# lbroseus/TALC

Measured on AMD Instinct MI355X. Metric: corrected long-read bases/sec (whole node); k-mer-probe HBM GB/s, higher is better.
Workload: dtype u8

## Files before the change

talc_amd/csrc/talc_capi.hip:

```cpp
#include <hip/hip_runtime.h>

#include <algorithm>
#include <atomic>
#include <chrono>
#include <cstdarg>
#include <cstdio>
#include <cstring>
#include <fstream>
#include <map>
#include <memory>
#include <mutex>
#include <sstream>
#include <string>
#include <vector>

#include "talc_common.h"
#include "talc_devmem.h"
#include "talc_hip.h"
#include "talc_kernels_build.h"
#include "talc_kernels_count.h"
#include "talc_kernels_edits.h"
#include "talc_kernels_pieces.h"
#include "talc_kernels_probe.h"
#include "talc_kernels_search.h"
// ... 910 lines not shown
}

int talc_ctx_get_map_timing(const talc_ctx* c, float* pack_map_ms, float* mask_case_ms) {
  if (!c) return fail(TALC_ERR_INVALID, "null context");
  if (pack_map_ms) *pack_map_ms = c->pack_map_ms;
  if (mask_case_ms) *mask_case_ms = c->mask_case_ms;
  return TALC_OK;
}

int talc_ctx_get_pieces_timing(const talc_ctx* c, float* count_ms, float* pack_ms) {
  if (!c) return fail(TALC_ERR_INVALID, "null context");
  if (count_ms) *count_ms = c->piece_count_ms;
  if (pack_ms) *pack_ms = c->piece_pack_ms;
  return TALC_OK;
}

int talc_ctx_get_solidity_timing(const talc_ctx* c, float* raw_ms, float* corrected_ms) {
  if (!c) return fail(TALC_ERR_INVALID, "null context");
  if (raw_ms) *raw_ms = c->sol_raw_ms;
  if (corrected_ms) *corrected_ms = c->sol_corr_ms;
  return TALC_OK;
}

int talc_ctx_get_timing(const talc_ctx* c, talc_timing* out) {
  if (!c || !out) return fail(TALC_ERR_INVALID, "null argument");
  *out = c->timing;
  return TALC_OK;
}

void talc_batch_destroy(talc_batch* b) { delete b; }

int talc_batch_create(talc_ctx* c, const char* bases, const uint64_t* offsets, uint32_t n_reads, talc_batch** out) {
  if (!c || !offsets || !out || (!bases && n_reads && offsets[n_reads] > 0)) return fail(TALC_ERR_INVALID, "null argument");
  HIPCHK(hipSetDevice(c->device));
  auto b = std::make_unique<talc_batch>();
  b->ctx = c; b->n_reads = n_reads;
  b->h_state.use_pool(&c->host_pool); b->h_dense_off.use_pool(&c->host_pool); b->h_seg_off.use_pool(&c->host_pool);
  b->h_offsets.assign(offsets, offsets + n_reads + 1);
  if (b->h_offsets[0] != 0) return fail(TALC_ERR_INVALID, "offsets[0] must be 0");
  b->n_bases = b->h_offsets[n_reads];
  const uint32_t K = c->p.k;
  b->h_koff.resize(n_reads + 1);
  b->h_regoff.resize(n_reads + 1);
  b->h_outoff.resize(n_reads + 1);
  uint64_t ko = 0, ro = 0, oo = 0;
  for (uint32_t r = 0; r < n_reads; ++r) {
    if (offsets[r + 1] < offsets[r]) return fail(TALC_ERR_INVALID, "offsets must be non-decreasing");
    const uint64_t L = offsets[r + 1] - offsets[r];
    if (L > 0x7fffff00ull) return fail(TALC_ERR_INVALID, "read %u too long", r);
    b->max_len = std::max<uint32_t>(b->max_len, (uint32_t)L);
    const uint64_t nk = L >= K ? L - K + 1 : 0;
    b->h_koff[r] = ko; ko += nk;
    b->h_regoff[r] = ro; ro += nk / 2 + 2;
    b->h_outoff[r] = oo; oo += out_capacity_for(L);
    for (uint64_t p = 0; p < nk; p += COV_TILE) { b->h_tile_read.push_back(r); b->h_tile_start.push_back((uint32_t)p); }
    for (uint64_t p = 0; p < L; p += 4096) { b->h_chunk_read.push_back(r); b->h_chunk_start.push_back((uint32_t)p); }
  }
  b->h_koff[n_reads] = ko; b->h_regoff[n_reads] = ro; b->h_outoff[n_reads] = oo;
  b->n_kmers = ko;
  hipStream_t s = c->stream;
  int rc;
  HIPCHK(b->d_raw.alloc(c->cache, std::max<uint64_t>(b->n_bases, 1)));
  HIPCHK(b->d_codes.alloc(c->cache, std::max<uint64_t>(b->n_bases, 1) + 64));
  if (b->n_bases) HIPCHK(hipMemcpyAsync(b->d_raw.get(), bases, b->n_bases, hipMemcpyHostToDevice, s));
  if ((rc = up(c, b->d_offsets, b->h_offsets, s))) return rc;
  if ((rc = up(c, b->d_koff, b->h_koff, s))) return rc;
  if ((rc = up(c, b->d_regoff, b->h_regoff, s))) return rc;
  if ((rc = up(c, b->d_outoff, b->h_outoff, s))) return rc;
  if ((rc = up(c, b->d_tile_read, b->h_tile_read, s))) return rc;
  if ((rc = up(c, b->d_tile_start, b->h_tile_start, s))) return rc;
  if ((rc = up(c, b->d_chunk_read, b->h_chunk_read, s))) return rc;
  if ((rc = up(c, b->d_chunk_start, b->h_chunk_start, s))) return rc;
  HIPCHK(b->d_order.alloc(c->cache, std::max<uint32_t>(n_reads, 1)));
  HIPCHK(b->d_cov.alloc(c->cache, std::max<uint64_t>(b->n_kmers, 1)));
  HIPCHK(b->d_covw.alloc(c->cache, cov_words_total(b->n_kmers, n_reads)));
  HIPCHK(b->d_nin.alloc(c->cache, std::max<uint32_t>(n_reads, 1)));
  HIPCHK(b->d_state.alloc(c->cache, std::max<uint32_t>(n_reads, 1)));
  HIPCHK(b->d_headcov.alloc(c->cache, std::max<uint32_t>(n_reads, 1) * (uint64_t)kHeadCov));
  HIPCHK(b->d_regions.alloc(c->cache, std::max<uint64_t>(ro, 1) * 3));
  HIPCHK(b->d_out.alloc(c->cache, std::max<uint64_t>(oo, 1)));
  HIPCHK(hipStreamSynchronize(s));
  *out = b.release();
  return TALC_OK;
}

uint64_t talc_batch_num_kmers(const talc_batch* b) { return b ? b->n_kmers : 0; }
uint64_t talc_batch_num_bases(const talc_batch* b) { return b ? b->n_bases : 0; }

static int launch_vote(talc_ctx* c, talc_batch* b) {
  HIPCHK(b->d_strand.ensure(c->cache, b->n_reads));
  HIPCHK(b->d_strand_flag.ensure(c->cache, b->n_reads));
  HIPCHK(hipEventRecord(c->ev[kEvVote0], c->stream));
  if (b->n_reads)
    hipLaunchKernelGGL(k_strand_vote, dim3(b->n_reads), dim3(64), 0, c->stream, c->view, b->d_raw.get(), b->d_offsets.get(), c->p.min_count, b->n_reads,
                       b->d_strand.get(), b->d_strand_flag.get());
  HIPCHK(hipGetLastError());
  HIPCHK(hipEventRecord(c->ev[kEvVote1], c->stream));
  c->votePending = true;
  b->holds.voted = true;
  return TALC_OK;
}
static int vote_time(talc_ctx* c) {
  if (!c->votePending) return TALC_OK;
  HIPCHK(hipEventElapsedTime(&c->vote_ms, c->ev[kEvVote0], c->ev[kEvVote1]));
  c->votePending = false;
  return TALC_OK;
}
// ... 700 lines not shown
```

talc_amd/csrc/talc_capi_correct.inc:

```

static uint32_t next_launch_stamp() {
  static std::atomic<uint32_t> launches{0};
  return 0x01000000u + (launches.fetch_add(1) & 0xFFFFFFu);
}
static void ensure_edge_boxes(talc_ctx* c, Stage& st) {
  const uint64_t gap = (uint64_t)c->p.max_border_length + 256;
  const uint32_t seqCap = (uint32_t)align_up((uint64_t)(2.2 * (double)gap) + 4ull * c->p.k + 64, 16);
  const uint64_t need = (uint64_t)st.n_slots * edge_box_bytes(seqCap) + (uint64_t)st.n_slots * 4;
  if (c->sw.edgeTasks == 0 || c->p.max_start_anchors < 2 || c->p.max_start_anchors > EDGE_BOX_ANCHORS ||
      seqCap > (1u << 16) || need > (1ull << 30)) {
    st.boxes.reset(); st.boxes_bytes = 0;
    return;
  }
  if (need > st.boxes_bytes || seqCap != st.box_seq_cap) {
    st.boxes.reset(); st.boxes_bytes = 0;
    if (st.boxes.alloc(need) != hipSuccess) { (void)hipGetLastError(); return; }
    st.boxes_bytes = need; st.box_seq_cap = seqCap;
  }
}

static int ensure_stage(talc_ctx* c, Stage& st, uint32_t maxLen, uint32_t scale, uint32_t n_work) {
  const SearchCaps caps = make_caps(maxLen, c->p.k, scale, scale == 1 ? c->sw.seqArena : 0, scale == 1 && c->sw.tinyCaps);
  hipDeviceProp_t prop;
  HIPCHK(hipGetDeviceProperties(&prop, c->device));
// ... 100 lines not shown
  hipStream_t s = c->stream;
  int rc;
  memset(&c->timing, 0, sizeof c->timing);
  c->timing.n_kmers = b->n_kmers; c->timing.n_bases = b->n_bases;
  if ((rc = prepare_strand(c, b))) return rc;
  HIPCHK(hipEventRecord(c->ev[kEvBegin], s));
  if (!b->holds.encoded && (rc = launch_encode(c, b))) return rc;
  HIPCHK(hipEventRecord(c->ev[kEvEncoded], s));
  if ((rc = launch_coverage(c, b))) return rc;
  HIPCHK(hipEventRecord(c->ev[kEvCovered], s));
  HIPCHK(hipMemsetAsync(batch_stats(c), 0, kBatchStatsWords * sizeof(uint32_t), s));
  if (b->n_reads)
    hipLaunchKernelGGL(k_structure, dim3(b->n_reads), dim3(64), 0, s, c->dp, c->view, b->d_codes.get(), b->d_offsets.get(), b->d_koff.get(),
                       b->d_cov.get(), b->d_covw.get(), b->d_nin.get(), b->d_state.get(), b->d_regions.get(), b->d_regoff.get(), b->d_headcov.get(), b->n_reads, tb, traceRead, batch_stats(c));
  HIPCHK(hipGetLastError());
  HIPCHK(hipEventRecord(c->ev[kEvStructured], s));
  return TALC_OK;
}

static int order_queue(talc_ctx* c, talc_batch* b) {
  if (!b->n_reads) return TALC_OK;
  hipStream_t s = c->stream;
  uint32_t* const hist = c->d_hist.get();
  HIPCHK(hipMemsetAsync(hist, 0, kOrderBuckets * sizeof(uint32_t), s));
  const unsigned nb = (b->n_reads + kOrderBlock - 1) / kOrderBlock;
  hipLaunchKernelGGL(k_order_scale, dim3(1), dim3(64), 0, s, batch_stats(c));
  hipLaunchKernelGGL(k_order_hist, dim3(nb), dim3(kOrderBlock), 0, s, b->d_state.get(), b->n_reads, hist, batch_stats(c));
  hipLaunchKernelGGL(k_order_scan, dim3(1), dim3(kOrderBuckets), 0, s, hist);
  hipLaunchKernelGGL(k_order_scatter, dim3(nb), dim3(kOrderBlock), 0, s, b->d_state.get(), b->n_reads, hist, b->d_order.get(), batch_stats(c));
  HIPCHK(hipGetLastError());
  return TALC_OK;
}

static int launch_search(talc_ctx* c, talc_batch* b, const Stage& st, const uint32_t* d_work, uint32_t n_work, const TraceBuf& tb,
                         uint32_t traceRead, bool edgeTasks) {
  hipStream_t s = c->stream;
  HIPCHK(hipMemsetAsync(c->d_queue.get(), 0, kQueueWords * sizeof(uint32_t), s));
  const memcheck::Setting poison = memcheck::setting();
  if (poison.on && st.scratch_bytes) HIPCHK(hipMemsetAsync(st.scratch.get(), poison.byte, st.scratch_bytes, s));
  EdgeTaskArgs ea = {};
  ea.test = c->sw.edgeLane ? 0u : kTestNoEdgeLane;
  if (edgeTasks && st.boxes) {
    ea.boxes = st.boxes.get();
    ea.avail = (uint32_t*)(st.boxes.get() + (uint64_t)st.n_slots * edge_box_bytes(st.box_seq_cap));
    ea.seqCap = st.box_seq_cap;
    ea.minWeak = c->sw.edgeTaskMin; ea.heavy = c->sw.edgeTaskHeavy; ea.heavyRounds = c->sw.edgeTaskRounds;
    ea.lingerMod = c->sw.edgeLingerMod; ea.test |= c->sw.edgeRedo ? kTestEdgeRedo : 0u;
    ea.autoSwitch = c->sw.edgeTasks > 0 ? nullptr : batch_stats(c) + kStatBranching;
    if (poison.on) HIPCHK(hipMemsetAsync(ea.boxes, poison.byte, (uint64_t)st.n_slots * edge_box_bytes(st.box_seq_cap), s));
    HIPCHK(hipMemsetAsync(ea.avail, 0, (uint64_t)st.n_slots * 4, s));
  }
  hipLaunchKernelGGL(k_search, dim3(st.n_slots), dim3(64), 0, s, c->dp, c->view, st.caps, b->d_codes.get(), b->d_offsets.get(),
                     b->d_koff.get(), b->d_cov.get(), b->d_covw.get(), b->d_state.get(), b->d_regions.get(), b->d_regoff.get(), b->d_headcov.get(),
                     c->map ? b->d_regions.get() : nullptr, c->map ? b->d_mapedge.get() : nullptr, b->d_out.get(), b->d_outoff.get(), d_work,
                     n_work, c->d_queue.get(), st.scratch.get(), c->d_counters.get(), tb, traceRead, next_launch_stamp(), ea);
  HIPCHK(hipGetLastError());
  return TALC_OK;
}

static int search_first_pass(talc_ctx* c, talc_batch* b, const TraceBuf& tb, uint32_t traceRead) {
  hipStream_t s = c->stream;
  int rc;
  HIPCHK(hipMemsetAsync(c->d_counters.get(), 0, kCounterWords * sizeof(uint64_t), s));
  HIPCHK(hipMemsetAsync(c->d_counters.get() + kCntFirstStart, 0xFF, sizeof(uint64_t), s));
  HIPCHK(hipMemsetAsync(c->d_counters.get() + kCntQueueDry, 0xFF, sizeof(uint64_t), s));
  if (b->n_reads) {
    if ((rc = ensure_stage(c, c->stage, b->max_len, 1, b->n_reads))) return rc;
    ensure_edge_boxes(c, c->stage);
    if ((rc = launch_search(c, b, c->stage, b->d_order.get(), b->n_reads, tb, traceRead, true))) return rc;
  }
  HIPCHK(hipEventRecord(c->ev[kEvSearched], s));
  return TALC_OK;
}

static int emit_offsets(talc_ctx* c, talc_batch* b, bool map, const uint64_t** totals) {
  hipStream_t s = c->stream;
  const uint32_t n = b->n_reads, nb = emit_blocks(n);
  HIPCHK(b->d_emit.ensure(c->cache, nb + 1));
  HIPCHK(b->d_dense_off.ensure(c->cache, n + 1));
  if (map) HIPCHK(b->d_seg_off.ensure(c->cache, n + 1));
  EmitSum* const sums = b->d_emit.get();
  hipLaunchKernelGGL(k_emit_sums, dim3(nb), dim3(kEmitThreads), 0, s, b->d_state.get(), n, sums);
  hipLaunchKernelGGL(k_emit_offsets, dim3(nb), dim3(kEmitThreads), 0, s, b->d_state.get(), n, sums, b->d_dense_off.get(),
                     map ? b->d_seg_off.get() : nullptr, (unsigned long long*)(sums + nb));
  HIPCHK(hipGetLastError());
  HIPCHK(hipMemcpyAsync(c->h_land.data(), sums + nb, kTotWords * sizeof(uint64_t), hipMemcpyDeviceToHost, s));
  HIPCHK(hipStreamSynchronize(s));
  *totals = c->h_land.data();
  return TALC_OK;
}

static int search_retry_passes(talc_ctx* c, talc_batch* b, const TraceBuf& tb, uint32_t traceRead) {
  hipStream_t s = c->stream;
  int rc;
  std::vector<uint32_t> retry;
  for (uint32_t r = 0; r < b->n_reads; ++r) if (b->h_state[r].overflow) retry.push_back(r);
  c->timing.n_retried = (uint32_t)retry.size();
  HIPCHK(hipEventRecord(c->ev[kEvRetry0], s));
  for (uint32_t scale = 8; scale <= 64 && !retry.empty(); scale *= 8) {
    Stage big;
    if ((rc = ensure_stage(c, big, b->max_len, scale, (uint32_t)retry.size()))) {
      if (rc == TALC_ERR_NOMEM) break;
      return rc;
    }
    DevBuf<uint32_t> d_retry;
    if (d_retry.alloc(retry.size()) != hipSuccess) { (void)hipGetLastError(); break; }
    HIPCHK(hipMemcpyAsync(d_retry.get(), retry.data(), retry.size() * 4, hipMemcpyHostToDevice, s));
    for (uint32_t r : retry) {
      b->h_state[r].overflow = 0;
      HIPCHK(hipMemcpyAsync(b->d_state.get() + r, &b->h_state[r], sizeof(ReadState), hipMemcpyHostToDevice, s));
    }
    if ((rc = launch_search(c, b, big, d_retry.get(), (uint32_t)retry.size(), tb, traceRead, false))) return rc;
    if ((rc = fetch_states(c, b))) return rc;
    d_retry.reset(); big = Stage();
    std::vector<uint32_t> again;
    for (uint32_t r : retry) if (b->h_state[r].overflow) again.push_back(r);
    retry.swap(again);
  }
  HIPCHK(hipEventRecord(c->ev[kEvRetry1], s));
  return TALC_OK;
}

static int pack_dense(talc_ctx* c, talc_batch* b, uint64_t total) {
  hipStream_t s = c->stream;
  HIPCHK(b->d_dense.ensure(c->cache, total));
  if (b->n_reads)
    hipLaunchKernelGGL(k_pack, dim3(b->n_reads), dim3(256), 0, s, b->d_out.get(), b->d_outoff.get(), b->d_state.get(), b->d_dense_off.get(), b->d_dense.get(),
                       b->n_reads, c->p.reverse ? 1 : 0, b->rev_flags());
  HIPCHK(hipGetLastError());
  HIPCHK(hipEventRecord(c->ev[kEvEmitted], s));
  return TALC_OK;
}

static int pack_map(talc_ctx* c, talc_batch* b, uint64_t total) {
  hipStream_t s = c->stream;
  HIPCHK(b->d_segs.ensure(c->cache, total));
  if (b->n_reads)
    hipLaunchKernelGGL(k_pack_map, dim3(b->n_reads), dim3(64), 0, s, b->d_state.get(), b->d_regions.get(), b->d_regoff.get(), b->d_mapedge.get(),
                       b->d_offsets.get(), b->d_seg_off.get(), b->d_segs.get(), b->n_reads, c->p.k, c->p.reverse ? 1 : 0,
                       b->rev_flags());
  HIPCHK(hipGetLastError());
  HIPCHK(hipEventRecord(c->ev[kEvPackMap], s));
  return TALC_OK;
}

static int read_timing(talc_ctx* c, talc_batch* b, bool map, uint32_t n_failed, const uint64_t** counters) {
  hipStream_t s = c->stream;
  const uint32_t n = b->n_reads;
  int rc;
  if (!b->h_state.resize(n) || !b->h_dense_off.resize(n + 1) || (map && !b->h_seg_off.resize(n + 1)))
    return fail(TALC_ERR_NOMEM, "cannot allocate the host copies of %u reads' states and offsets", n);
  uint64_t* const land = c->h_land.data() + kTotWords;
  if (n) HIPCHK(hipMemcpyAsync(b->h_state.data(), b->d_state.get(), (size_t)n * sizeof(ReadState), hipMemcpyDeviceToHost, s));
  HIPCHK(hipMemcpyAsync(b->h_dense_off.data(), b->d_dense_off.get(), ((size_t)n + 1) * 8, hipMemcpyDeviceToHost, s));
  if (map) HIPCHK(hipMemcpyAsync(b->h_seg_off.data(), b->d_seg_off.get(), ((size_t)n + 1) * 8, hipMemcpyDeviceToHost, s));
  HIPCHK(hipMemcpyAsync(land, c->d_counters.get(), kCntWaveLog * sizeof(uint64_t), hipMemcpyDeviceToHost, s));
  HIPCHK(hipStreamSynchronize(s));
  if ((rc = read_stage_times(c, kEvEmitted))) return rc;
  c->timing.n_trail_steps = land[kCntSteps];
  c->timing.n_dp_cells = land[kCntCells];
  c->timing.n_failed = n_failed;
  if (c->sw.timing)
    fprintf(stderr, "[talc-lib] correction: host arrays page-locked: states %d, offsets %d, landing area %d\n", b->h_state.pinned() ? 1 : 0,
            b->h_dense_off.pinned() ? 1 : 0, c->h_land.pinned() ? 1 : 0);
  *counters = land;
  return TALC_OK;
}

static int run_pipeline(talc_ctx* c, talc_batch* b, TraceHost* th, uint32_t traceRead) {
  HIPCHK(hipSetDevice(c->device));
  int rc;
  b->holds.drop_results();
  const bool map = c->map;
  if (map) HIPCHK(b->d_mapedge.ensure(c->cache, 2ull * std::max<uint32_t>(b->n_reads, 1)));
  const TraceBuf tb = trace_buf(c, th);
  const uint64_t* counters = nullptr;
  const uint64_t* tot = nullptr;
  if ((rc = launch_structure(c, b, tb, traceRead))) return rc;
  if ((rc = order_queue(c, b))) return rc;
  if ((rc = search_first_pass(c, b, tb, traceRead))) return rc;
  HIPCHK(hipEventRecord(c->ev[kEvRetry0], c->stream));
  HIPCHK(hipEventRecord(c->ev[kEvRetry1], c->stream));
  if ((rc = emit_offsets(c, b, map, &tot))) return rc;
  if (tot[kTotOverflow]) {
    if ((rc = fetch_states(c, b))) return rc;
    if ((rc = search_retry_passes(c, b, tb, traceRead))) return rc;
    if ((rc = emit_offsets(c, b, map, &tot))) return rc;
  }
  const uint32_t n_failed = (uint32_t)tot[kTotOverflow];
  if ((rc = pack_dense(c, b, tot[kTotBytes]))) return rc;
  if (map && (rc = pack_map(c, b, tot[kTotSegs]))) return rc;
  if ((rc = read_timing(c, b, map, n_failed, &counters)) || (rc = vote_time(c))) return rc;
  if (map) HIPCHK(hipEventElapsedTime(&c->pack_map_ms, c->ev[kEvEmitted], c->ev[kEvPackMap]));
#ifdef TALC_PROF
  if ((rc = prof_report(c, b, counters))) return rc;
#endif
  b->holds.corrected = true; b->holds.mapped = map;
  if (c->timing.n_failed) {
    fail(TALC_WARN_READ_ERRORS, "%u read(s) exhausted the device scratch even in the retry pass (status TALC_READ_ERROR)", c->timing.n_failed);
    return TALC_WARN_READ_ERRORS;
  }
  return TALC_OK;
}

int talc_batch_correct(talc_ctx* c, talc_batch* b) {
  if (int rc = belong(c, b, "bad context/batch")) return rc;
  return run_pipeline(c, b, nullptr, 0xFFFFFFFFu);
}

int talc_batch_structure(talc_ctx* c, talc_batch* b) {
  int rc;
  if ((rc = enter(c, b, "bad context/batch"))) return rc;
  b->holds.drop_results();
  if ((rc = launch_structure(c, b, TraceBuf{}, 0xFFFFFFFFu))) return rc;
  if ((rc = fetch_states(c, b))) return rc;
  if ((rc = read_stage_times(c, kEvStructured)) || (rc = vote_time(c))) return rc;
  b->holds.structured = true;
  return TALC_OK;
}

int talc_batch_order(talc_ctx* c, talc_batch* b, uint32_t* order, uint32_t* bucket) {
  if (int rc = belong(c, b, "bad context/batch/buffer", order && bucket)) return rc;
  if (!b->holds.structured) return fail(TALC_ERR_STATE, "talc_batch_structure has not run on this batch (or a correction has run since)");
  HIPCHK(hipSetDevice(c->device));
  int rc;
  if ((rc = order_queue(c, b))) return rc;
  uint32_t scale = 256u;
// ... 346 lines not shown
```

talc_amd/csrc/talc_kernels_search.h:

```cpp
#pragma once
#include "talc_common.h"
#include "talc_kernels_probe.h"
#include "talc_pure.h"
#include "talc_wave.h"

namespace talc {

#define TCAP 320
#define NBUF 576
static_assert(TCAP >= 64 + 4 * 60 - 1 && NBUF % 64 == 0 && NBUF >= 4 * 60 + 64 + 4 * 60 - 1,
              "TCAP and NBUF cover gardening's kept list at the largest accepted parameters (check_params)");
#ifndef LDS_DP_CAP
#define LDS_DP_CAP 320
#endif
#ifndef HOT
#define HOT 8
#endif
#ifndef AIMS_LDS
#define AIMS_LDS 16
#endif

enum : uint32_t {
  OVF_ANCHORS = 1, OVF_FULLPATHS = 2, OVF_FULLPOOL = 4, OVF_TRAILS = 8, OVF_SEQ = 16, OVF_OUT = 32, OVF_WEAKPOOL = 64,
  OVF_REGIONS = 128, OVF_DP = 256
// ... 3443 lines not shown
    X.LH = X.regH[reg]; X.RH = X.regH[reg + 1];
    X.weakLen = (X.Rs > X.Le + K) ? (X.Rs - (X.Le + K)) : 0;
    if (attempt == 0) { build_anchors(0); build_anchors(1); }
    if (uni((int)X.tracing)) trace_search_cold();
    PROF_BEGIN2(); success = search_bridge(wo, wl, weakUsed); PROF_END2(PF_SRCHB);
    if (uni((int)X.tracing)) {
      if (success) trace_rec(TR_RESULT, 1, 1, (int)X.Le, (int)X.Rs, 0.0, X.weak + wo, wl, false);
      else trace_rec(TR_RESULT, 1, 0, (int)X.regE[reg], (int)X.regS[reg + 1], 0.0, X.read + X.regE[reg] + K, X.weakLen, false);
    }
  }
  WSYNC();
  if (success && lane_id() == 0) { X.regE[reg] = X.Le; X.regH[reg + 1] += X.Rs - X.regS[reg + 1]; X.regS[reg + 1] = X.Rs; X.wOff[reg] = wo; X.wLen[reg] = wl; }
  WSYNC();
}

template <int LOC>
TALC_D void correct_border(Piece& border, uint32_t R, uint32_t& weakUsed, SearchProf& pf) {
  constexpr bool HEAD = (LOC == LOC_HEAD);
  const uint32_t reg = HEAD ? 0 : R - 1;
  PROF_DECL2;
  X.location = LOC; X.dirRight = HEAD ? 0 : 1;
  if (HEAD) { X.Rs = X.regS[reg]; X.Re = X.regE[reg]; X.Ls = 0; X.Le = 0; X.RH = X.regH[reg]; X.LH = 0; X.weakLen = X.Rs; X.nAncL = 0; }
  else { X.Ls = X.regS[reg]; X.Le = X.regE[reg]; X.Rs = 0; X.Re = 0; X.LH = X.regH[reg]; X.RH = 0; X.weakLen = X.L - (X.Le + X.P.K); X.nAncR = 0; }
  build_anchors(HEAD ? 1 : 0);
  if (uni((int)X.tracing)) trace_search_cold();
  uint32_t off = 0, len = 0;
  PROF_BEGIN2(); pf.edge_begins(); const bool found = search_edge(off, len, weakUsed); pf.edge_ends(); PROF_END2(PF_SRCHE);
  if (uni((int)X.tracing)) {
    if (found) trace_rec(TR_RESULT, LOC, 1, HEAD ? 0 : (int)X.Le, HEAD ? (int)X.Rs : 0, 0.0, X.weak + off, len, false);
    else trace_rec(TR_RESULT, LOC, 0, HEAD ? 0 : (int)X.regE[reg], HEAD ? (int)X.regS[reg] : 0, 0.0, border.p, X.weakLen, false);
  }
  WSYNC();
  if (found && lane_id() == 0) {
    if (HEAD) { X.regH[reg] += X.Rs - X.regS[reg]; X.regS[reg] = X.Rs; }
    else X.regE[reg] = X.Le;
  }
  WSYNC();
  if (found) border = uni_piece(X.weak + off, len);
}

TALC_D Piece piece_after(uint32_t i, uint32_t R, uint32_t K) {
  if (i + 1 >= R) return Piece{nullptr, 0};
  if (X.wLen[i] != kNotCorrected) return Piece{X.weak + X.wOff[i], X.wLen[i]};
  const uint32_t from = X.regE[i] + K, to = X.regS[i + 1];
  return Piece{X.read + from, to > from ? to - from : 0};
}

TALC_D unsigned long long corrected_length(const Piece& head, const Piece& tail, uint32_t R) {
  const uint32_t K = X.P.K;
  unsigned long long part = 0;
  for (uint32_t i = lane_id(); i < R; i += 64) part += (unsigned long long)X.regE[i] + K - X.regS[i] + piece_after(i, R, K).n;
  return head.n + wave_sum_u64(part) + tail.n;
}
TALC_D void reassemble(uint8_t* out, const Piece& head, const Piece& tail, uint32_t R, ReadState* rs) {
  const uint32_t K = X.P.K;
  uint32_t pos = 0;
  auto put = [&](const uint8_t* p, uint32_t n) { copy_bytes(out + pos, p, n, false); pos += n; };
  if (head.n) put(head.p, head.n);
  for (uint32_t i = 0; i < R; ++i) {
    const uint32_t s = X.regS[i];
    put(X.read + s, X.regE[i] + K - s);
    const Piece w = piece_after(i, R, K);
    if (w.n) put(w.p, w.n);
  }
  if (tail.n) put(tail.p, tail.n);
  unsigned long long part = 0;
  for (uint32_t i = lane_id(); i < R; i += 64) part += (unsigned long long)X.regE[i] - X.regS[i] + 1;
  const uint32_t span = (uint32_t)wave_sum_u64(part);
  if (lane_id() == 0) { rs->outLen = pos; rs->inSpan = span; }
}

TALC_D void leave_outcome(uint32_t r, const Piece& head, const Piece& tail, uint32_t R, uint32_t* regions, const uint64_t* regoff,
                          uint32_t* mapEdge) {
  uint32_t* gS = regions + 3 * regoff[r];
  const uint32_t gCap = (uint32_t)(regoff[r + 1] - regoff[r]);
  uint32_t* gE = gS + gCap;
  uint32_t* gW = gE + gCap;
  for (uint32_t i = lane_id(); i < R; i += 64) { gS[i] = X.regS[i]; gE[i] = X.regE[i]; gW[i] = X.wLen[i]; }
  if (lane_id() == 0) {
    mapEdge[2ull * r] = (head.p == X.read) ? kNotCorrected : head.n;
    mapEdge[2ull * r + 1] = (tail.p + tail.n == X.read + X.L) ? kNotCorrected : tail.n;
  }
}

TALC_D void pass_through(uint8_t* out, ReadState* rs, uint32_t overflow) {
  copy_bytes(out, X.read, X.L, false);
  if (lane_id() == 0) { rs->outLen = X.L; if (overflow) rs->overflow = overflow; }
}

#ifndef TALC_SEARCH_WAVES_PER_SIMD
#define TALC_SEARCH_WAVES_PER_SIMD 5
#endif
__global__ void __launch_bounds__(64, TALC_SEARCH_WAVES_PER_SIMD)
k_search(DevParams P, TableView T, SearchCaps C, const uint8_t* __restrict__ codes, const uint64_t* __restrict__ offsets,
         const uint64_t* __restrict__ koff, const uint2* __restrict__ covAll, const CovWord* __restrict__ covWords,
         ReadState* __restrict__ state,
         const uint32_t* regions, const uint64_t* __restrict__ regoff, const uint32_t* __restrict__ headCovAll,
         uint32_t* mapRegions, uint32_t* __restrict__ mapEdge,
         uint8_t* __restrict__ outAll,
         const uint64_t* __restrict__ outoff, const uint32_t* __restrict__ order, uint32_t n_work,
         uint32_t* __restrict__ queue, uint8_t* __restrict__ scratchAll, uint64_t* __restrict__ counters, TraceBuf trace,
         uint32_t traceRead, uint32_t launchStamp, EdgeTaskArgs E) {
  __shared__ uint32_t s_next;
  const int l = lane_id();
  bind_slot(scratchAll + (uint64_t)blockIdx.x * C.slotBytes, C, trace);
  const uint32_t lingerMod = bind_launch(P, T, queue, n_work, launchStamp, E);
  X.mapRegions = mapRegions; X.mapEdge = mapEdge;
  unsigned long long totCells = 0, totSteps = 0;
  PROF_DECL2;
  SearchProf pf;
  pf.wave_begins();

  while (true) {
    WSYNC();
    pf.read_ends(state);
    if (X.boxes != nullptr) edge_between_reads();
    if (l == 0) s_next = atomicAdd(queue, 1u);
    WSYNC();
    const uint32_t qi = s_next;
    if (qi >= n_work) break;
    X.qi = qi;
    PROF_BEGIN2();
    const uint32_t r = order[qi];
    pf.read_begins(state, qi, r);
    ReadState* const rs = state + r;
    uint8_t* out = outAll + outoff[r];
    const uint32_t outCap = (uint32_t)(outoff[r + 1] - outoff[r]);
    const ReadState st = *rs;
    if (!begin_read(r, st, C.regCap, codes, offsets, koff, covAll, covWords, headCovAll, regions, regoff, trace, traceRead)) { pass_through(out, rs, 0u); continue; }
    const uint32_t R = st.nRegions;
    uint32_t weakUsed = 0;
    PROF_END2(PF_PROLOG);
    Piece head = {nullptr, 0}, tail = head;
    if (!X.overflow) {
      const uint32_t tailLen = X.L - (X.regE[R - 1] + P.K);
      head = uni_piece(X.read, X.regS[0]); tail = uni_piece(X.read + (X.L - tailLen), tailLen);
      for (uint32_t reg = 0; reg + 1 < R && !X.overflow; ++reg) correct_inner(reg, weakUsed);
      if (!X.overflow && head.n > 0 && head.n <= P.MAX_BORDER_LEN) correct_border<LOC_HEAD>(head, R, weakUsed, pf);
      if (!X.overflow && tail.n > 0 && tail.n <= P.MAX_BORDER_LEN) correct_border<LOC_TAIL>(tail, R, weakUsed, pf);
    }
    totCells += X.cells; totSteps += X.steps;
    pf.read_searched(state);
    if (X.overflow) { pass_through(out, rs, X.overflow); continue; }
    if (corrected_length(head, tail, R) > outCap) { pass_through(out, rs, OVF_OUT); continue; }
    PROF_BEGIN2();
    reassemble(out, head, tail, R, rs);
    if (uni_ptr(X.mapEdge) != nullptr) leave_outcome(r, head, tail, R, uni_ptr(X.mapRegions), regoff, uni_ptr(X.mapEdge));
    PROF_END2(PF_ASSEMBLE);
  }
  pf.queue_dry(counters);
  if (X.boxes != nullptr && blockIdx.x % lingerMod == 0u) pf.lingered(edge_linger(n_work));
  totCells += X.moreCells; totSteps += X.moreSteps;
  if (l == 0) {
    if (totSteps) atomicAdd((unsigned long long*)&counters[kCntSteps], totSteps);
    if (totCells) atomicAdd((unsigned long long*)&counters[kCntCells], totCells);
    pf.wave_ends(state, counters);
  }
}

static_assert(kOrderBuckets == 32 * 32, "the key of order_bucket: five bits of exponent, five of mantissa");
__host__ __device__ inline uint32_t order_bucket(const ReadState& st, uint32_t gapScale) {
  if (st.status != TALC_READ_CORRECTED || st.overflow) return kOrderBuckets - 1;
  return order_key_bucket(st.costEst, st.costGap, gapScale, kOrderBuckets);
}
__global__ void __launch_bounds__(64) k_order_scale(uint32_t* __restrict__ batchStats) {
  const int l = lane_id();
  const unsigned long long fork = wave_sum_u64(batchStats[2 * l]), solid = wave_sum_u64(batchStats[2 * l + 1]);
  uint32_t scale = 256u;
  if (solid > 0) {
    const unsigned long long perMille10 = fork * 10000ull / solid;
    if (perMille10 > 120ull) scale = 256u + (uint32_t)min((perMille10 - 120ull) * 256ull / 100ull, 512ull);
  }
  if (l == 0) { batchStats[kStatGapScale] = scale; batchStats[kStatBranching] = scale > 256u ? 1u : 0u; }
}
static const uint32_t kOrderBlock = kOrderBuckets;
__global__ void __launch_bounds__(kOrderBlock)
k_order_hist(const ReadState* __restrict__ state, uint32_t n, uint32_t* __restrict__ hist, const uint32_t* __restrict__ batchStats) {
  __shared__ uint32_t cnt[kOrderBuckets];
  const uint32_t t = threadIdx.x, r = blockIdx.x * kOrderBlock + t;
  cnt[t] = 0u;
  __syncthreads();
  if (r < n) atomicAdd(&cnt[order_bucket(state[r], batchStats[kStatGapScale])], 1u);
  __syncthreads();
  if (cnt[t]) atomicAdd(&hist[t], cnt[t]);
}
__global__ void __launch_bounds__(kOrderBuckets) k_order_scan(uint32_t* __restrict__ hist) {
  __shared__ uint32_t s[kOrderBuckets];
  const uint32_t t = threadIdx.x;
  const uint32_t v = hist[t];
  s[t] = v;
  __syncthreads();
  for (uint32_t off = 1; off < kOrderBuckets; off <<= 1) {
    const uint32_t add = (t >= off) ? s[t - off] : 0u;
    __syncthreads();
    s[t] += add;
    __syncthreads();
  }
  hist[t] = s[t] - v;
}
__global__ void __launch_bounds__(kOrderBlock)
// ... 49 lines not shown
#pragma unroll
  for (int off = 1; off < 64; off <<= 1) {
    const unsigned long long t = ((unsigned long long)(uint32_t)__shfl_up((int)(incl >> 32), off, 64) << 32) | (uint32_t)__shfl_up((int)(uint32_t)incl, off, 64);
    if (l >= (uint32_t)off) incl += t;
  }
  __syncthreads();
  if (l == 63u) waveSums[w] = incl;
  __syncthreads();
  unsigned long long before = 0;
  total = 0;
  for (uint32_t i = 0; i < kEmitThreads / 64; ++i) { const unsigned long long s = waveSums[i]; if (i < w) before += s; total += s; }
  return before + incl - v;
}
__global__ void __launch_bounds__(kEmitThreads)
k_emit_offsets(const ReadState* __restrict__ state, uint32_t n, const EmitSum* __restrict__ blockSums, uint64_t* __restrict__ denseOff,
               uint64_t* __restrict__ segOff, unsigned long long* __restrict__ totals) {
  __shared__ unsigned long long waveSums[kEmitThreads / 64];
  EmitSum carry = {0, 0, 0};
  for (uint32_t i = threadIdx.x; i < blockIdx.x; i += kEmitThreads) { const EmitSum e = blockSums[i]; carry.bytes += e.bytes; carry.segs += e.segs; carry.ovf += e.ovf; }
  carry = EmitSum{emit_block_sum(carry.bytes, waveSums), emit_block_sum(carry.segs, waveSums), emit_block_sum(carry.ovf, waveSums)};
  EmitSum mine = {0, 0, 0};
  const uint32_t r0 = blockIdx.x * kEmitReads + threadIdx.x * kEmitPer;
  for (uint32_t i = 0; i < kEmitPer; ++i)
    if (r0 + i < n) { const EmitSum e = emit_read(state[r0 + i]); mine.bytes += e.bytes; mine.segs += e.segs; mine.ovf += e.ovf; }
  EmitSum tot;
  unsigned long long bytesAt = carry.bytes + emit_block_scan(mine.bytes, waveSums, tot.bytes);
  unsigned long long segsAt = carry.segs + emit_block_scan(mine.segs, waveSums, tot.segs);
  tot.ovf = emit_block_sum(mine.ovf, waveSums);
  for (uint32_t i = 0; i < kEmitPer && r0 + i < n; ++i) {
    const EmitSum e = emit_read(state[r0 + i]);
    denseOff[r0 + i] = bytesAt; if (segOff) segOff[r0 + i] = segsAt;
    bytesAt += e.bytes; segsAt += e.segs;
  }
  if (blockIdx.x + 1 == gridDim.x && threadIdx.x == 0) {
    denseOff[n] = carry.bytes + tot.bytes;
    if (segOff) segOff[n] = carry.segs + tot.segs;
    totals[kTotOverflow] = carry.ovf + tot.ovf; totals[kTotBytes] = carry.bytes + tot.bytes; totals[kTotSegs] = carry.segs + tot.segs;
  }
}

__global__ void k_build_thresholds(double ALPHA, uint32_t n, uint32_t* __restrict__ thr) {
  const uint32_t c = blockIdx.x * blockDim.x + threadIdx.x;
  if (c >= n) return;
  uint32_t lo = 0, hi = 0x7FFFFFFFu;
  if (!is_expected_by_model(ALPHA, hi, c, false)) lo = hi = 0xFFFFFFFFu;
  while (lo < hi) { const uint32_t mid = lo + (hi - lo) / 2; if (is_expected_by_model(ALPHA, mid, c, false)) hi = mid; else lo = mid + 1; }
  thr[2u * c] = lo;
  lo = 0; hi = 0x7FFFFFFFu;
  if (is_expected_by_model(ALPHA, hi, c, true)) lo = hi = 0xFFFFFFFFu;
  while (lo < hi) { const uint32_t mid = lo + (hi - lo) / 2; if (!is_expected_by_model(ALPHA, mid, c, true)) hi = mid; else lo = mid + 1; }
  thr[2u * c + 1u] = lo;
}

TALC_D uint32_t codes4_to_ascii(uint32_t w, bool complement) {
  if (w & 0xF8F8F8F8u) {
    uint32_t o = 0;
    for (int i = 0; i < 4; ++i) {
      const uint8_t c = (uint8_t)(w >> (8 * i));
      o |= (uint32_t)(uint8_t)code_to_ascii(complement ? complement_code(c) : c) << (8 * i);
    }
    return o;
  }
  return __builtin_amdgcn_perm(0x4E4E4E4Eu, complement ? 0x41434754u : 0x54474341u, w);
}
__global__ void __launch_bounds__(256)
k_pack(const uint8_t* __restrict__ outAll, const uint64_t* __restrict__ outoff, const ReadState* __restrict__ state,
       const uint64_t* __restrict__ dense_off, uint8_t* __restrict__ dense, uint32_t n_reads, int reverse,
       const uint8_t* __restrict__ rev_flags) {
  const uint32_t r = blockIdx.x;
  if (r >= n_reads) return;
  if (rev_flags) reverse |= rev_flags[r];
  const uint8_t* src = outAll + outoff[r];
  const uint32_t len = state[r].outLen;
  uint8_t* dst = dense + dense_off[r];
  const bool rc = reverse && state[r].status == TALC_READ_CORRECTED && state[r].overflow == 0;
  const uint32_t t = threadIdx.x, T = blockDim.x;
  const uint32_t head = min(len, (uint32_t)((4u - ((uintptr_t)dst & 3u)) & 3u));
  const uint32_t nw = (len - head) / 4u;
  uint32_t* const dw = (uint32_t*)(dst + head);
  if (!rc) {
    const uint32_t sh = (uint32_t)(((uintptr_t)src + head) & 3u);
    const uint32_t* const sw = (const uint32_t*)(src + head - sh);
    for (uint32_t w = t; w < nw; w += T) {
      const uint32_t lo = sw[w], hi = sh ? sw[w + 1] : 0u;
      dw[w] = codes4_to_ascii((uint32_t)((((uint64_t)hi << 32) | lo) >> (8u * sh)), false);
    }
  } else if (nw) {
    const uint8_t* const top = src + (len - head - 4u);
    const uint32_t sh = (uint32_t)((uintptr_t)top & 3u);
    const uint32_t* const sw = (const uint32_t*)(top - sh);
    for (uint32_t w = t; w < nw; w += T) {
      const uint32_t* const at = sw - w;
      const uint32_t lo = at[0], hi = sh ? at[1] : 0u;
      dw[w] = codes4_to_ascii(__builtin_bswap32((uint32_t)((((uint64_t)hi << 32) | lo) >> (8u * sh))), true);
    }
  }
  const uint32_t done = head + 4u * nw;
  for (uint32_t i = t; i < head + (len - done); i += T) {
    const uint32_t at = i < head ? i : done + (i - head);
    dst[at] = rc ? (uint8_t)code_to_ascii(complement_code(src[len - 1 - at])) : (uint8_t)code_to_ascii(src[at]);
  }
}

struct MapSeg { uint32_t kind, rawStart, rawLen, outStart, outLen; };
enum : uint32_t { SEG_SOLID = 0, SEG_CORRECTED = 1, SEG_RAW = 2 };
__global__ void __launch_bounds__(64)
k_pack_map(const ReadState* __restrict__ state, const uint32_t* __restrict__ regions, const uint64_t* __restrict__ regoff,
           const uint32_t* __restrict__ mapEdge, const uint64_t* __restrict__ offsets, const uint64_t* __restrict__ segOff,
           MapSeg* __restrict__ segs, uint32_t n_reads, uint32_t K, int reverse, const uint8_t* __restrict__ rev_flags) {
  const uint32_t r = blockIdx.x;
  if (r >= n_reads) return;
  if (rev_flags) reverse |= rev_flags[r];
  const uint32_t l = (uint32_t)lane_id();
  const uint32_t L = (uint32_t)(offsets[r + 1] - offsets[r]);
  const ReadState st = state[r];
  MapSeg* const o = segs + segOff[r];
  if (!map_has_outcome(st)) {
    if (l == 0) o[0] = MapSeg{SEG_RAW, 0u, L, 0u, L};
    return;
  }
  const uint32_t R = st.nRegions, nseg = 2 * R + 1, outLen = st.outLen;
  const uint32_t* gS = regions + 3 * regoff[r];
  const uint32_t gCap = (uint32_t)(regoff[r + 1] - regoff[r]);
  const uint32_t* gE = gS + gCap;
  const uint32_t* gW = gE + gCap;
  uint32_t carry = 0;
  for (uint32_t base = 0; base < nseg; base += 64) {
    const uint32_t j = base + l;
    MapSeg s = {SEG_RAW, 0u, 0u, 0u, 0u};
    if (j < nseg) {
      uint32_t w = kNotCorrected;
      if (j == 0) { s.rawLen = gS[0]; w = mapEdge[2ull * r]; }
      else if (j == 2 * R) { s.rawStart = gE[R - 1] + K; s.rawLen = L - s.rawStart; w = mapEdge[2ull * r + 1]; }
      else {
        const uint32_t i = (j - 1) >> 1;
        if (j & 1u) { s.kind = SEG_SOLID; s.rawStart = gS[i]; s.rawLen = gE[i] + K - s.rawStart; }
        else { const uint32_t to = gS[i + 1]; s.rawStart = gE[i] + K; s.rawLen = to > s.rawStart ? to - s.rawStart : 0u; w = gW[i]; }
      }
      s.outLen = s.rawLen;
      if (w != kNotCorrected) { s.kind = SEG_CORRECTED; s.outLen = w; }
    }
    uint32_t incl = s.outLen;
#pragma unroll
    for (int off = 1; off < 64; off <<= 1) { const uint32_t t = (uint32_t)__shfl_up((int)incl, off, 64); if (l >= (uint32_t)off) incl += t; }
    s.outStart = carry + incl - s.outLen;
    carry += (uint32_t)__shfl((int)incl, 63, 64);
    if (j < nseg) {
      if (reverse) { s.rawStart = L - s.rawStart - s.rawLen; s.outStart = outLen - s.outStart - s.outLen; o[nseg - 1 - j] = s; }
      else o[j] = s;
    }
  }
}

__global__ void __launch_bounds__(256)
k_mask_case(const MapSeg* __restrict__ segs, const uint64_t* __restrict__ segOff, const uint64_t* __restrict__ dense_off,
            uint8_t* __restrict__ masked, uint32_t n_reads) {
  const uint32_t r = blockIdx.x;
  if (r >= n_reads) return;
  uint8_t* const rec = masked + dense_off[r];
  const uint32_t recLen = (uint32_t)(dense_off[r + 1] - dense_off[r]);
  for (uint64_t k = segOff[r]; k < segOff[r + 1]; ++k) {
    const MapSeg s = segs[k];
    if (s.kind != SEG_RAW) continue;
    for (uint32_t i = threadIdx.x; i < s.outLen && s.outStart + i < recLen; i += blockDim.x) rec[s.outStart + i] |= 0x20u;
  }
}

__global__ void __launch_bounds__(64, TALC_SEARCH_WAVES_PER_SIMD)
k_test_dp(int mode, const uint8_t* a, int la, const uint8_t* b, int lb, int p0, int p1, int p2, int p3, int K,
          int* dpG, uint32_t dpCap, int* out, double alpha, double err, int minc, const uint32_t* thr, uint32_t thrN) {
  if (lane_id() == 0) memset(&g_X, 0, sizeof g_X);
  WSYNC();
  X.P.K = (uint32_t)K; X.P.ALPHA = alpha; X.P.ERR = err; X.P.MIN_COUNT = (uint32_t)minc;
  X.C.dpCap = dpCap; X.dpG = dpG;
  X.dirRight = p1;
  if (mode == 0) {
    const int r = nw_score(a, la, b, lb, p0, p1, p2, p3 != 0);
    if (lane_id() == 0) { out[0] = r; out[5] = (int)X.overflow; }
  } else if (mode == 1) {
    const SeedExt e = seed_and_extension(a, la, b, lb, p0, true);
    if (lane_id() == 0) { out[0] = e.lenRefExt; out[1] = e.lenHistExt; out[2] = e.posOnRef; out[3] = e.score; out[4] = e.stop ? 1 : 0; out[5] = (int)X.overflow; }
  } else if (mode == 2) {
    const int r = wave_find_window(a, la, b, lb, p3 != 0);
    if (lane_id() == 0) out[0] = r;
  } else if (mode == 5) {
    int* rc_ = X.dpG; int* rr_ = X.dpG + X.C.dpCap; int* rs_ = X.dpG + 2ull * X.C.dpCap;
    const bool ok = seed_and_extension_multi(a, la, b, lb, p0, rc_, rr_, rs_);
    int nbad = 0, first = -1;
    const int S5 = X.dirRight ? K - 1 : K;
    const bool sameAnchor = ballot64(lane_id() < S5 && lane_id() < la && lane_id() < lb && a[lane_id() < la ? lane_id() : 0] != b[lane_id() < lb ? lane_id() : 0]) == 0ull && la >= S5 && lb >= S5;
    if (ok) {
      for (int x = 0; x <= p0; ++x) {
        const SeedExt m = seedext_plain(la, lb, uni(rc_[x]), uni(rr_[x]), x);
        const int msc = uni(rs_[x]);
// ... 94 lines not shown
```

Before: 4.892 billion.

## Gather packed output from raw read and weak pieces instead of reassembling in search

The search kernel no longer copies the full corrected read (solid regions plus corrected pieces) into the per-read output buffer. It only copies the compact weak-piece bytes, and always records region and edge outcome data even when not in map mode. k_pack now rebuilds each output on the fly: it scans the segments, binary-searches which segment each output position falls in, and reads either from the original codes or from the piece buffer. This drops a full per-read copy from the latency-heavy search kernel, at the cost of more complex indexed gathers in k_pack and extra metadata writes.

```diff
diff --git a/talc_amd/csrc/talc_capi.hip b/talc_amd/csrc/talc_capi.hip
--- a/talc_amd/csrc/talc_capi.hip
+++ b/talc_amd/csrc/talc_capi.hip
@@ -986,7 +986,7 @@
     const uint64_t nk = L >= K ? L - K + 1 : 0;
     b->h_koff[r] = ko; ko += nk;
     b->h_regoff[r] = ro; ro += nk / 2 + 2;
-    b->h_outoff[r] = oo; oo += out_capacity_for(L);
+    b->h_outoff[r] = oo; oo += align_up(out_capacity_for(L), 16);
     for (uint64_t p = 0; p < nk; p += COV_TILE) { b->h_tile_read.push_back(r); b->h_tile_start.push_back((uint32_t)p); }
     for (uint64_t p = 0; p < L; p += 4096) { b->h_chunk_read.push_back(r); b->h_chunk_start.push_back((uint32_t)p); }
   }
diff --git a/talc_amd/csrc/talc_capi_correct.inc b/talc_amd/csrc/talc_capi_correct.inc
--- a/talc_amd/csrc/talc_capi_correct.inc
+++ b/talc_amd/csrc/talc_capi_correct.inc
@@ -176,7 +176,7 @@
   }
   hipLaunchKernelGGL(k_search, dim3(st.n_slots), dim3(64), 0, s, c->dp, c->view, st.caps, b->d_codes.get(), b->d_offsets.get(),
                      b->d_koff.get(), b->d_cov.get(), b->d_covw.get(), b->d_state.get(), b->d_regions.get(), b->d_regoff.get(), b->d_headcov.get(),
-                     c->map ? b->d_regions.get() : nullptr, c->map ? b->d_mapedge.get() : nullptr, b->d_out.get(), b->d_outoff.get(), d_work,
+                     b->d_regions.get(), b->d_mapedge.get(), b->d_out.get(), b->d_outoff.get(), d_work,
                      n_work, c->d_queue.get(), st.scratch.get(), c->d_counters.get(), tb, traceRead, next_launch_stamp(), ea);
   HIPCHK(hipGetLastError());
   return TALC_OK;
@@ -249,7 +249,8 @@
   hipStream_t s = c->stream;
   HIPCHK(b->d_dense.ensure(c->cache, total));
   if (b->n_reads)
-    hipLaunchKernelGGL(k_pack, dim3(b->n_reads), dim3(256), 0, s, b->d_out.get(), b->d_outoff.get(), b->d_state.get(), b->d_dense_off.get(), b->d_dense.get(),
+    hipLaunchKernelGGL(k_pack, dim3(b->n_reads), dim3(kPackThreads), 0, s, b->d_codes.get(), b->d_offsets.get(), b->d_regions.get(), b->d_regoff.get(),
+                       b->d_mapedge.get(), c->p.k, b->d_out.get(), b->d_outoff.get(), b->d_state.get(), b->d_dense_off.get(), b->d_dense.get(),
                        b->n_reads, c->p.reverse ? 1 : 0, b->rev_flags());
   HIPCHK(hipGetLastError());
   HIPCHK(hipEventRecord(c->ev[kEvEmitted], s));
@@ -296,7 +297,7 @@
   int rc;
   b->holds.drop_results();
   const bool map = c->map;
-  if (map) HIPCHK(b->d_mapedge.ensure(c->cache, 2ull * std::max<uint32_t>(b->n_reads, 1)));
+  HIPCHK(b->d_mapedge.ensure(c->cache, 2ull * std::max<uint32_t>(b->n_reads, 1)));
   const TraceBuf tb = trace_buf(c, th);
   const uint64_t* counters = nullptr;
   const uint64_t* tot = nullptr;
diff --git a/talc_amd/csrc/talc_kernels_search.h b/talc_amd/csrc/talc_kernels_search.h
--- a/talc_amd/csrc/talc_kernels_search.h
+++ b/talc_amd/csrc/talc_kernels_search.h
@@ -3519,22 +3519,12 @@
   for (uint32_t i = lane_id(); i < R; i += 64) part += (unsigned long long)X.regE[i] + K - X.regS[i] + piece_after(i, R, K).n;
   return head.n + wave_sum_u64(part) + tail.n;
 }
-TALC_D void reassemble(uint8_t* out, const Piece& head, const Piece& tail, uint32_t R, ReadState* rs) {
-  const uint32_t K = X.P.K;
-  uint32_t pos = 0;
-  auto put = [&](const uint8_t* p, uint32_t n) { copy_bytes(out + pos, p, n, false); pos += n; };
-  if (head.n) put(head.p, head.n);
-  for (uint32_t i = 0; i < R; ++i) {
-    const uint32_t s = X.regS[i];
-    put(X.read + s, X.regE[i] + K - s);
-    const Piece w = piece_after(i, R, K);
-    if (w.n) put(w.p, w.n);
-  }
-  if (tail.n) put(tail.p, tail.n);
+TALC_D void leave_pieces(uint8_t* out, uint32_t weakUsed, uint32_t outLen, uint32_t R, ReadState* rs) {
+  wave_copy(uni_ptr(out), uni_ptr(X.weak), (uint32_t)uni((int)weakUsed));
   unsigned long long part = 0;
   for (uint32_t i = lane_id(); i < R; i += 64) part += (unsigned long long)X.regE[i] - X.regS[i] + 1;
   const uint32_t span = (uint32_t)wave_sum_u64(part);
-  if (lane_id() == 0) { rs->outLen = pos; rs->inSpan = span; }
+  if (lane_id() == 0) { rs->outLen = outLen; rs->inSpan = span; }
 }
 
 TALC_D void leave_outcome(uint32_t r, const Piece& head, const Piece& tail, uint32_t R, uint32_t* regions, const uint64_t* regoff,
@@ -3550,8 +3540,7 @@
   }
 }
 
-TALC_D void pass_through(uint8_t* out, ReadState* rs, uint32_t overflow) {
-  copy_bytes(out, X.read, X.L, false);
+TALC_D void pass_through(ReadState* rs, uint32_t overflow) {
   if (lane_id() == 0) { rs->outLen = X.L; if (overflow) rs->overflow = overflow; }
 }
 
@@ -3592,9 +3581,8 @@
     pf.read_begins(state, qi, r);
     ReadState* const rs = state + r;
     uint8_t* out = outAll + outoff[r];
-    const uint32_t outCap = (uint32_t)(outoff[r + 1] - outoff[r]);
     const ReadState st = *rs;
-    if (!begin_read(r, st, C.regCap, codes, offsets, koff, covAll, covWords, headCovAll, regions, regoff, trace, traceRead)) { pass_through(out, rs, 0u); continue; }
+    if (!begin_read(r, st, C.regCap, codes, offsets, koff, covAll, covWords, headCovAll, regions, regoff, trace, traceRead)) { pass_through(rs, 0u); continue; }
     const uint32_t R = st.nRegions;
     uint32_t weakUsed = 0;
     PROF_END2(PF_PROLOG);
@@ -3608,11 +3596,12 @@
     }
     totCells += X.cells; totSteps += X.steps;
     pf.read_searched(state);
-    if (X.overflow) { pass_through(out, rs, X.overflow); continue; }
-    if (corrected_length(head, tail, R) > outCap) { pass_through(out, rs, OVF_OUT); continue; }
+    if (X.overflow) { pass_through(rs, X.overflow); continue; }
+    const unsigned long long outLen = corrected_length(head, tail, R);
+    if (outLen > (uint32_t)out_capacity_for(X.L)) { pass_through(rs, OVF_OUT); continue; }
     PROF_BEGIN2();
-    reassemble(out, head, tail, R, rs);
-    if (uni_ptr(X.mapEdge) != nullptr) leave_outcome(r, head, tail, R, uni_ptr(X.mapRegions), regoff, uni_ptr(X.mapEdge));
+    leave_pieces(out, weakUsed, (uint32_t)outLen, R, rs);
+    leave_outcome(r, head, tail, R, uni_ptr(X.mapRegions), regoff, uni_ptr(X.mapEdge));
     PROF_END2(PF_ASSEMBLE);
   }
   pf.queue_dry(counters);
@@ -3768,6 +3757,30 @@
   thr[2u * c + 1u] = lo;
 }
 
+struct MapSeg { uint32_t kind, rawStart, rawLen, outStart, outLen; };
+enum : uint32_t { SEG_SOLID = 0, SEG_CORRECTED = 1, SEG_RAW = 2 };
+struct ReadOutcome { const uint32_t* gS; const uint32_t* gE; const uint32_t* gW; uint32_t headW, tailW, R, K, L; };
+TALC_D ReadOutcome read_outcome(uint32_t r, uint32_t R, uint32_t K, uint32_t L, const uint32_t* __restrict__ regions,
+                                const uint64_t* __restrict__ regoff, const uint32_t* __restrict__ mapEdge) {
+  const uint32_t* gS = regions + 3 * regoff[r];
+  const uint32_t gCap = (uint32_t)(regoff[r + 1] - regoff[r]);
+  return ReadOutcome{gS, gS + gCap, gS + 2ull * gCap, mapEdge[2ull * r], mapEdge[2ull * r + 1], R, K, L};
+}
+TALC_D MapSeg outcome_segment(const ReadOutcome& o, uint32_t j) {
+  MapSeg s = {SEG_RAW, 0u, 0u, 0u, 0u};
+  uint32_t w = kNotCorrected;
+  if (j == 0) { s.rawLen = o.gS[0]; w = o.headW; }
+  else if (j == 2 * o.R) { s.rawStart = o.gE[o.R - 1] + o.K; s.rawLen = o.L - s.rawStart; w = o.tailW; }
+  else {
+    const uint32_t i = (j - 1) >> 1;
+    if (j & 1u) { s.kind = SEG_SOLID; s.rawStart = o.gS[i]; s.rawLen = o.gE[i] + o.K - s.rawStart; }
+    else { const uint32_t to = o.gS[i + 1]; s.rawStart = o.gE[i] + o.K; s.rawLen = to > s.rawStart ? to - s.rawStart : 0u; w = o.gW[i]; }
+  }
+  s.outLen = s.rawLen;
+  if (w != kNotCorrected) { s.kind = SEG_CORRECTED; s.outLen = w; }
+  return s;
+}
+
 TALC_D uint32_t codes4_to_ascii(uint32_t w, bool complement) {
   if (w & 0xF8F8F8F8u) {
     uint32_t o = 0;
@@ -3779,47 +3792,98 @@
   }
   return __builtin_amdgcn_perm(0x4E4E4E4Eu, complement ? 0x41434754u : 0x54474341u, w);
 }
-__global__ void __launch_bounds__(256)
-k_pack(const uint8_t* __restrict__ outAll, const uint64_t* __restrict__ outoff, const ReadState* __restrict__ state,
+static const uint32_t kPackThreads = 64, kPackSegs = kPackThreads;
+TALC_D uint32_t codes4_at(const uint8_t* s) {
+  const uint32_t sh = (uint32_t)((uintptr_t)s & 3u);
+  const uint32_t* const w = (const uint32_t*)(s - sh);
+  const uint32_t lo = w[0], hi = sh ? w[1] : 0u;
+  return (uint32_t)((((uint64_t)hi << 32) | lo) >> (8u * sh));
+}
+template <class Word, class Code>
+TALC_D void pack_stretch(uint8_t* dst, uint32_t len, bool rc, uint32_t a, uint32_t b, Word word, Code code) {
+  const uint32_t t = threadIdx.x;
+  const uint32_t pa = rc ? len - b : a, n = b - a;
+  const uint32_t head = min(n, (uint32_t)((4u - ((uintptr_t)(dst + pa) & 3u)) & 3u));
+  const uint32_t nw = (n - head) / 4u;
+  uint32_t* const dw = (uint32_t*)(dst + pa + head);
+  for (uint32_t w = t; w < nw; w += kPackThreads) {
+    const uint32_t p = pa + head + 4u * w;
+    dw[w] = rc ? codes4_to_ascii(__builtin_bswap32(word(len - p - 4u)), true) : codes4_to_ascii(word(p), false);
+  }
+  const uint32_t done = head + 4u * nw;
+  for (uint32_t i = t; i < n - 4u * nw; i += kPackThreads) {
+    const uint32_t p = pa + (i < head ? i : done + (i - head));
+    dst[p] = rc ? (uint8_t)code_to_ascii(complement_code(code(len - 1u - p))) : (uint8_t)code_to_ascii(code(p));
+  }
+}
+__global__ void __launch_bounds__(kPackThreads)
+k_pack(const uint8_t* __restrict__ codes, const uint64_t* __restrict__ offsets, const uint32_t* __restrict__ regions,
+       const uint64_t* __restrict__ regoff, const uint32_t* __restrict__ mapEdge, uint32_t K,
+       const uint8_t* __restrict__ outAll, const uint64_t* __restrict__ outoff, const ReadState* __restrict__ state,
        const uint64_t* __restrict__ dense_off, uint8_t* __restrict__ dense, uint32_t n_reads, int reverse,
        const uint8_t* __restrict__ rev_flags) {
+  __shared__ uint32_t sStart[kPackSegs + 1];
+  __shared__ uint32_t sSrc[kPackSegs];
+  __shared__ uint8_t sPiece[kPackSegs];
   const uint32_t r = blockIdx.x;
   if (r >= n_reads) return;
   if (rev_flags) reverse |= rev_flags[r];
-  const uint8_t* src = outAll + outoff[r];
-  const uint32_t len = state[r].outLen;
-  uint8_t* dst = dense + dense_off[r];
-  const bool rc = reverse && state[r].status == TALC_READ_CORRECTED && state[r].overflow == 0;
-  const uint32_t t = threadIdx.x, T = blockDim.x;
-  const uint32_t head = min(len, (uint32_t)((4u - ((uintptr_t)dst & 3u)) & 3u));
-  const uint32_t nw = (len - head) / 4u;
-  uint32_t* const dw = (uint32_t*)(dst + head);
-  if (!rc) {
-    const uint32_t sh = (uint32_t)(((uintptr_t)src + head) & 3u);
-    const uint32_t* const sw = (const uint32_t*)(src + head - sh);
-    for (uint32_t w = t; w < nw; w += T) {
-      const uint32_t lo = sw[w], hi = sh ? sw[w + 1] : 0u;
-      dw[w] = codes4_to_ascii((uint32_t)((((uint64_t)hi << 32) | lo) >> (8u * sh)), false);
-    }
-  } else if (nw) {
-    const uint8_t* const top = src + (len - head - 4u);
-    const uint32_t sh = (uint32_t)((uintptr_t)top & 3u);
-    const uint32_t* const sw = (const uint32_t*)(top - sh);
-    for (uint32_t w = t; w < nw; w += T) {
-      const uint32_t* const at = sw - w;
-      const uint32_t lo = at[0], hi = sh ? at[1] : 0u;
-      dw[w] = codes4_to_ascii(__builtin_bswap32((uint32_t)((((uint64_t)hi << 32) | lo) >> (8u * sh))), true);
-    }
-  }
-  const uint32_t done = head + 4u * nw;
-  for (uint32_t i = t; i < head + (len - done); i += T) {
-    const uint32_t at = i < head ? i : done + (i - head);
-    dst[at] = rc ? (uint8_t)code_to_ascii(complement_code(src[len - 1 - at])) : (uint8_t)code_to_ascii(src[at]);
-  }
-}
-
-struct MapSeg { uint32_t kind, rawStart, rawLen, outStart, outLen; };
-enum : uint32_t { SEG_SOLID = 0, SEG_CORRECTED = 1, SEG_RAW = 2 };
+  const ReadState st = state[r];
+  const uint8_t* const read = codes + offsets[r];
+  const uint32_t len = st.outLen;
+  uint8_t* const dst = dense + dense_off[r];
+  const bool rc = reverse && st.status == TALC_READ_CORRECTED && st.overflow == 0;
+  if (!map_has_outcome(st)) {
+    pack_stretch(dst, len, rc, 0u, len, [&](uint32_t c) { return codes4_at(read + c); }, [&](uint32_t c) { return read[c]; });
+    return;
+  }
+  const uint8_t* const pieces = outAll + outoff[r];
+  const uint32_t t = threadIdx.x;
+  const ReadOutcome o = read_outcome(r, st.nRegions, K, (uint32_t)(offsets[r + 1] - offsets[r]), regions, regoff, mapEdge);
+  const uint32_t R = o.R, nseg = 2 * R + 1;
+  unsigned long long mine = 0;
+  for (uint32_t i = t; i + 1 < R; i += kPackThreads) { const uint32_t w = o.gW[i]; mine += w != kNotCorrected ? w : 0u; }
+  const uint32_t headAt = (uint32_t)wave_sum_u64(mine);
+  const uint32_t tailAt = headAt + (o.headW != kNotCorrected ? o.headW : 0u);
+  uint32_t outCarry = 0, pieceCarry = 0;
+  for (uint32_t base = 0; base < nseg; base += kPackSegs) {
+    const uint32_t j = base + t, n = min(kPackSegs, nseg - base);
+    MapSeg s = {SEG_RAW, 0u, 0u, 0u, 0u};
+    if (j < nseg) s = outcome_segment(o, j);
+    const bool piece = s.kind == SEG_CORRECTED, between = piece && j != 0 && j != 2 * R;
+    const unsigned long long v = ((unsigned long long)(between ? s.outLen : 0u) << 32) | s.outLen;
+    unsigned long long incl = v;
+#pragma unroll
+    for (int off = 1; off < 64; off <<= 1) {
+      const unsigned long long up = ((unsigned long long)(uint32_t)__shfl_up((int)(incl >> 32), off, 64) << 32) | (uint32_t)__shfl_up((int)(uint32_t)incl, off, 64);
+      if (t >= (uint32_t)off) incl += up;
+    }
+    const unsigned long long at = incl - v;
+    const unsigned long long tot = ((unsigned long long)(uint32_t)__shfl((int)(incl >> 32), 63, 64) << 32) | (uint32_t)__shfl((int)(uint32_t)incl, 63, 64);
+    sStart[t] = outCarry + (uint32_t)at;
+    sSrc[t] = !piece ? s.rawStart : j == 0 ? headAt : j == 2 * R ? tailAt : pieceCarry + (uint32_t)(at >> 32);
+    sPiece[t] = piece ? 1 : 0;
+    const uint32_t a = min(outCarry, len), b = min(outCarry + (uint32_t)tot, len);
+    if (t == 0) sStart[kPackSegs] = outCarry + (uint32_t)tot;
+    outCarry += (uint32_t)tot; pieceCarry += (uint32_t)(tot >> 32);
+    WSYNC();
+    auto segment_of = [&](uint32_t c) {
+      uint32_t lo = 0, hi = n;
+      while (hi - lo > 1u) { const uint32_t mid = (lo + hi) >> 1; if (sStart[mid] <= c) lo = mid; else hi = mid; }
+      return lo;
+    };
+    auto source = [&](uint32_t g, uint32_t c) { return (sPiece[g] ? pieces : read) + sSrc[g] + (c - sStart[g]); };
+    auto code = [&](uint32_t c) { return *source(segment_of(c), c); };
+    auto word = [&](uint32_t c) {
+      const uint32_t g = segment_of(c);
+      if (c + 4u <= sStart[g + 1]) return codes4_at(source(g, c));
+      return (uint32_t)code(c) | (uint32_t)code(c + 1) << 8 | (uint32_t)code(c + 2) << 16 | (uint32_t)code(c + 3) << 24;
+    };
+    pack_stretch(dst, len, rc, a, b, word, code);
+    WSYNC();
+  }
+}
+
 __global__ void __launch_bounds__(64)
 k_pack_map(const ReadState* __restrict__ state, const uint32_t* __restrict__ regions, const uint64_t* __restrict__ regoff,
            const uint32_t* __restrict__ mapEdge, const uint64_t* __restrict__ offsets, const uint64_t* __restrict__ segOff,
@@ -3836,26 +3900,12 @@
     return;
   }
   const uint32_t R = st.nRegions, nseg = 2 * R + 1, outLen = st.outLen;
-  const uint32_t* gS = regions + 3 * regoff[r];
-  const uint32_t gCap = (uint32_t)(regoff[r + 1] - regoff[r]);
-  const uint32_t* gE = gS + gCap;
-  const uint32_t* gW = gE + gCap;
+  const ReadOutcome oc = read_outcome(r, R, K, L, regions, regoff, mapEdge);
   uint32_t carry = 0;
   for (uint32_t base = 0; base < nseg; base += 64) {
     const uint32_t j = base + l;
     MapSeg s = {SEG_RAW, 0u, 0u, 0u, 0u};
-    if (j < nseg) {
-      uint32_t w = kNotCorrected;
-      if (j == 0) { s.rawLen = gS[0]; w = mapEdge[2ull * r]; }
-      else if (j == 2 * R) { s.rawStart = gE[R - 1] + K; s.rawLen = L - s.rawStart; w = mapEdge[2ull * r + 1]; }
-      else {
-        const uint32_t i = (j - 1) >> 1;
-        if (j & 1u) { s.kind = SEG_SOLID; s.rawStart = gS[i]; s.rawLen = gE[i] + K - s.rawStart; }
-        else { const uint32_t to = gS[i + 1]; s.rawStart = gE[i] + K; s.rawLen = to > s.rawStart ? to - s.rawStart : 0u; w = gW[i]; }
-      }
-      s.outLen = s.rawLen;
-      if (w != kNotCorrected) { s.kind = SEG_CORRECTED; s.outLen = w; }
-    }
+    if (j < nseg) s = outcome_segment(oc, j);
     uint32_t incl = s.outLen;
 #pragma unroll
     for (int off = 1; off < 64; off <<= 1) { const uint32_t t = (uint32_t)__shfl_up((int)incl, off, 64); if (l >= (uint32_t)off) incl += t; }
```

New measurement: 4.932 billion, median of 6. About the same (+0.8%).
